# piotrkawa/audio-deepfake-adversarial-attacks

Hardware: AMD Instinct MI355X
Metric: adversarial utterances/sec, PGD-40 LCNN+LFCC 4s@16kHz (higher is better)
Workload: dtype f32

## Files before the change

### audio_deepfake_adversarial_attacks_amd/_lib.py

```python
from __future__ import annotations

import ctypes
from pathlib import Path

import os

_LIB_PATH = Path(os.environ.get("ADVSTEP_LIB") or Path(__file__).resolve().parent / "libadvstep.so")
_lib = None

OK, EINVAL, EWORKSPACE, ELAUNCH, ENODEVICE = 0, 1, 2, 3, 4
ABI_VERSION = 3

_p, _i64, _f32, _f64, _u64, _sz = (ctypes.c_void_p, ctypes.c_int64, ctypes.c_float, ctypes.c_double,
                                   ctypes.c_uint64, ctypes.c_size_t)

SIGNATURES = {
    "advstep_abi_version": (ctypes.c_int, []),
    "advstep_status_string": (ctypes.c_char_p, [ctypes.c_int]),
    "advstep_device_count": (ctypes.c_int, []),
    "advstep_row_workspace_bytes": (_sz, [_i64, _i64]),
    "advstep_minmax_normalize_f32": (ctypes.c_int, [_p, _p, _p, _p, _i64, _i64, _p, _sz, _p]),
    "advstep_minmax_revert_f32": (ctypes.c_int, [_p, _p, _p, _p, _i64, _i64, _p]),
    "advstep_fgsm_step_f32": (ctypes.c_int, [_p, _p, _p, _i64, _f32, _f32, _f32, _p]),
    "advstep_pgd_linf_init_noise_f32": (ctypes.c_int, [_p, _p, _p, _i64, _f32, _f32, _p]),
    "advstep_pgd_linf_init_philox_f32": (ctypes.c_int, [_p, _p, _i64, _f32, _f32, _f32, _u64, _u64, _p]),
# ... 24 lines not shown
    "advstep_lstm_backward_f32": (ctypes.c_int, [_p, _p, _p, _p, _p, _i64, _i64, _i64, _i64, _p]),
    "advstep_lstm_backward_bcast_f32": (ctypes.c_int, [_p, _p, _p, _p, _p, _i64, _i64, _i64, _i64, _p]),
    "advstep_lstm_backward_outer_f32": (ctypes.c_int, [_p, _p, _p, _p, _p, _p, _i64, _i64, _i64, _i64, _p]),
    "advstep_lcnn_tail_pack_f32": (ctypes.c_int, [_p, _p, _i64, _i64, _i64, _i64, _p]),
    "advstep_lcnn_tail_forward_f32": (ctypes.c_int, [_p, _p, _p, _p, _p, _i64, _i64, _i64, _p]),
    "advstep_lcnn_tail_unpack_add_f32": (ctypes.c_int, [_p, _p, _p, _i64, _i64, _i64, _i64, _p]),
    "advstep_lcnn_tail_unpack_add_outer_f32": (ctypes.c_int, [_p, _p, _p, _p, _i64, _i64, _i64, _i64, _p]),
    "advstep_gru_supported": (ctypes.c_int, [_i64]),
    "advstep_gru_forward_f32": (ctypes.c_int, [_p, _p, _p, _p, _p, _i64, _i64, _i64, _i64, _p]),
    "advstep_gru_backward_f32": (ctypes.c_int, [_p, _p, _p, _p, _p, _i64, _i64, _i64, _i64, _p]),
    "advstep_conv3x3_supported": (ctypes.c_int, [_i64, _i64]),
    "advstep_conv3x3_prepared_floats": (_sz, [_i64, _i64, ctypes.c_int]),
    "advstep_conv3x3_prepare_f32": (ctypes.c_int, [_p, _p, _p, _i64, _i64, ctypes.c_int, _p]),
    "advstep_conv3x3_mfm_pool2_forward_f32": (ctypes.c_int, [_p, _p, _p, _p, _p, _p, _p, _i64, _i64, _i64, _i64, _i64, _p]),
    "advstep_conv3x3_mfm_pool2_backward_f32": (ctypes.c_int, [_p, _p, _p, _p, _i64, _i64, _i64, _i64, _i64, _p]),
    "advstep_conv3x3_mfm_sel_bytes": (_sz, [_i64, _i64, _i64, _i64]),
    "advstep_conv3x3_mfm_forward_f32": (ctypes.c_int, [_p, _p, _p, _p, _p, _p, _p, _i64, _i64, _i64, _i64, _i64, _p]),
    "advstep_conv3x3_mfm_backward_f32": (ctypes.c_int, [_p, _p, _p, _p, _i64, _i64, _i64, _i64, _p]),
    "advstep_conv3x3_backward_data_f32": (ctypes.c_int, [_p, _p, _p, _i64, _i64, _i64, _i64, _i64, _p]),
    "advstep_afms_row_f32": (ctypes.c_int, [ctypes.c_int, _p, _p, _p, _p, _p, _p, _i64, _i64, _i64, _p]),
    "advstep_gate_maxpool2_backward_gate_f32": (ctypes.c_int, [_p, _p, _p, _p, _i64, _i64, _i64, _i64, _p]),
    "advstep_gate_maxpool2_backward_input_f32": (ctypes.c_int, [_p, _p, _p, _p, _p, _i64, _i64, _i64, _i64, _p]),
    "advstep_weighted_stats_forward_f32": (ctypes.c_int, [_p, _p, _p, _p, _i64, _i64, _p]),
    "advstep_weighted_stats_backward_f32": (ctypes.c_int, [_p, _p, _p, _p, _p, _p, _i64, _i64, _p]),
    "advstep_log_meannorm_max_length": (ctypes.c_int, []),
    "advstep_log_meannorm_forward_f32": (ctypes.c_int, [_p, ctypes.c_float, _p, _i64, _i64, _p]),
    "advstep_log_meannorm_backward_f32": (ctypes.c_int, [_p, _p, ctypes.c_float, _p, _i64, _i64, _p]),
    "advstep_tail_pool1d_forward_f32": (ctypes.c_int, [_p, _p, _p, _p, _p, _p, _p, _i64, _i64, _i64, _i64, _p]),
    "advstep_tail_pool1d_backward_f32": (ctypes.c_int, [_p, _p, _p, _p, _p, _p, _p, _i64, _i64, _i64, _i64, _p]),
    "advstep_res2net_link_forward_f32": (ctypes.c_int, [_p, _p, _p, _p, _p, _i64, _p, _i64, _p, _i64, _i64, _i64, _p]),
# ... 129 lines not shown
```

### audio_deepfake_adversarial_attacks_amd/csrc/advstep.hip

```cpp

#include <hip/hip_runtime.h>
#include <atomic>
#include <math.h>
#include <stdint.h>
#include <stdlib.h>

#include "advstep.h"
#include "advstep_common.h"
#include "row_tiles.h"

namespace {

constexpr int kMaxGrid = 256 * 16;

__device__ __forceinline__ float fgsm_elem(float x, float g, float eps, float lo, float hi) {
    return clampf(x + eps * sgn(g), lo, hi);
}

__device__ __forceinline__ float pgd_linf_elem(float a, float g, float x, float alpha, float eps, float lo,
                                               float hi) {
    a = a + alpha * sgn(g);
    float d = clampf(a - x, -eps, eps);
    return clampf(x + d, lo, hi);
}
// ... 790 lines not shown
                hipLaunchKernelGGL((KERNEL<false>), dim3(C_, (unsigned)nb_), dim3(kWgThreads), 0, st, __VA_ARGS__); \
        }                                                                                                  \
    } while (0)

extern "C" {

int advstep_abi_version(void) { return ADVSTEP_ABI_VERSION; }

const char *advstep_status_string(int status) {
    switch (status) {
        case ADVSTEP_OK: return "ok";
        case ADVSTEP_EINVAL: return "invalid argument";
        case ADVSTEP_EWORKSPACE: return "row workspace missing, misaligned or too small";
        case ADVSTEP_ELAUNCH: return "HIP kernel launch failed";
        case ADVSTEP_ENODEVICE: return "no HIP device";
        default: return "unknown status";
    }
}

int advstep_device_count(void) {
    int n = 0;
    if (hipGetDeviceCount(&n) != hipSuccess) {
        (void)hipGetLastError();
        return 0;
    }
    return n;
}

size_t advstep_row_workspace_bytes(int64_t B, int64_t T) {
    if (B <= 0 || T <= 0) return 0;
// ... 257 lines not shown
```

### audio_deepfake_adversarial_attacks_amd/csrc/lcnn_wino.hip

```cpp

#include <hip/hip_runtime.h>
#include <math.h>
#include <stdint.h>
#include <stdlib.h>

#include <type_traits>

#include "advstep_detector.h"
#include "advstep_lcnn.h"
#include "advstep_common.h"
#include "lcnn_wino_plan.h"

namespace {

extern __shared__ __attribute__((aligned(16))) float wino_u_s[];
__shared__ __attribute__((aligned(16))) float wino_cst[48];
__shared__ float wino_few_w[64];

__device__ __forceinline__ void weight_transform(const float (&g)[3][3], float (&u)[4][4]) {
    float t[4][3];
#pragma unroll
    for (int b = 0; b < 3; ++b) {
        t[0][b] = g[0][b];
        t[1][b] = 0.5f * (g[0][b] + g[1][b] + g[2][b]);
        t[2][b] = 0.5f * (g[0][b] - g[1][b] + g[2][b]);
        t[3][b] = g[2][b];
    }
#pragma unroll
    for (int a = 0; a < 4; ++a) {
        u[a][0] = t[a][0];
        u[a][1] = 0.5f * (t[a][0] + t[a][1] + t[a][2]);
        u[a][2] = 0.5f * (t[a][0] - t[a][1] + t[a][2]);
// ... 126 lines not shown
#pragma unroll
            for (int i = 0; i < kChunkFloats / 4 / kThreads; ++i) dst[threadIdx.x + i * kThreads] = src[threadIdx.x + i * kThreads];
        }
    }
    __device__ __forceinline__ void landed() const {
        if (DMA) __builtin_amdgcn_s_waitcnt(0x0F70);
    }
    __device__ __forceinline__ const float *a_ptr(int s, int buf, int g, int nl) const {
        return wino_u_s + buf * kChunkFloats + (((s & 3) * 4 + g) * 16 + nl) * 2;
    }
};

template <Epi EPI>
__device__ __forceinline__ void stage_constants(int slice, int Cout, const float *bias, const float *bn_mean,
                                                const float *bn_invstd, const GenArgs &ga) {
    if (adds_few(EPI) && threadIdx.x >= 64 && threadIdx.x < 128) {
        const float *w1x1 = bn_mean;
        const int i = threadIdx.x - 64, row = i >> 1, c = i & 1, ch = slice * 32 + row;
        wino_few_w[i] = (ch < Cout && c < ga.few) ? w1x1[ch * ga.few + c] : 0.0f;
    }
    if (has_constants(EPI) && threadIdx.x < 48) {
        const int q = threadIdx.x >> 4, j = threadIdx.x & 15;
        float v = q == 2 ? 1.0f : 0.0f;
        if (is_mfm(EPI)) {
            const int ch = slice * 16 + j;
            if (ch < Cout) {
                if (q == 2) v = bn_mean ? bn_invstd[ch] : 1.0f;
                else v = (bias ? bias[ch + q * Cout] : 0.0f) - (bn_mean ? bn_mean[ch] : 0.0f);
            }
        } else if (q < 2) {
// ... 20 lines not shown
        v[a4][2] = tr[a4][2] - tr[a4][1];
        v[a4][3] = tr[a4][1] - tr[a4][3];
    }
}

template <Epi EPI, bool STREAM, Src SRC, int NT = 2, bool GEN = false, bool WODD = false>
__global__ __launch_bounds__(kThreads) void wino3x3_kernel(const float *__restrict__ x, const uint8_t *__restrict__ xsel,
                                                           const float *__restrict__ U,
                                                           const float *__restrict__ bias,
                                                           const float *__restrict__ bn_mean,
                                                           const float *__restrict__ bn_invstd, float *__restrict__ y,
                                                           EpiBytes<EPI> *__restrict__ idx, int N, int K, int H, int W, int Cout,
                                                           int slices, int ranges, int slice0, GenArgs ga) {
    static_assert(NT == 2 || plain_store(EPI), "one accumulator tile only for the plain-store epilogues");
    static_assert(!GEN || SRC != Src::MfmPooled, "the general reduction reads dense tensors or a plain pooled gradient");
    const WgPlace wg = place_of_workgroup<NT>(slices, ranges, slice0, ga);
    const int half = wg.half, slice = wg.slice, range = wg.range;
    const int chunks = (K + kChunkCin - 1) / kChunkCin, steps = K / 4;
    const float *Usl = U + (int64_t)slice * chunks * kChunkFloats;
    const WeightChunks<STREAM && chunks_by_dma(SRC)> wc{Usl};
    constexpr bool kHasConst = has_constants(EPI);
    stage_constants<EPI>(slice, Cout, bias, bn_mean, bn_invstd, ga);
    if (!STREAM) {
        for (int c = 0; c < chunks; ++c) wc.copy(c, c);
    }
    if (!STREAM || kHasConst) __syncthreads();
    const int wave = threadIdx.x >> 6, lane = threadIdx.x & 63, g = lane >> 4, nl = lane & 15;
    const int TH = (H + 1) >> 1, TW = (W + 1) >> 1;
    const int tiles = N * TH * TW, groups = (tiles + 15) >> 4;
    const int iters = (groups + ranges * kWaves - 1) / (ranges * kWaves);
    const uint32_t plane = (uint32_t)(H * W);
    const int Hs = H >> 1, Ws = W >> 1, Cs = SRC == Src::MfmPooled ? K >> 1 : (GEN ? ga.Kreal : K);
    const uint32_t cplane = (uint32_t)(Hs * Ws);
    const int KA = GEN ? ga.K1 : K, KB = GEN ? ga.Kreal - ga.K1 : 0;
    const size_t src_elems = SRC == Src::Dense ? (size_t)N * KA * plane : (size_t)N * Cs * cplane;
    const __amdgpu_buffer_rsrc_t xr =
        __builtin_amdgcn_make_buffer_rsrc(const_cast<float *>(x), 0, (int)(src_elems * 4), 0x00020000);
    const __amdgpu_buffer_rsrc_t xr2 = __builtin_amdgcn_make_buffer_rsrc(
        const_cast<float *>(GEN && KB > 0 ? ga.x2 : x), 0, GEN && KB > 0 ? (int)((size_t)N * KB * plane * 4) : 0, 0x00020000);
    const __amdgpu_buffer_rsrc_t sr =
        __builtin_amdgcn_make_buffer_rsrc(const_cast<uint8_t *>(SRC != Src::Dense ? xsel : reinterpret_cast<const uint8_t *>(x)), 0,
// ... 238 lines not shown
                    }
                }
        }
        uint32_t hb[reads_sign_bytes(EPI) ? 4 : 1][reads_sign_bytes(EPI) ? NT : 1];
        if constexpr (reads_sign_bytes(EPI)) {
            const uint8_t *act = idx;
#pragma unroll
            for (int r = 0; r < 4; ++r)
#pragma unroll
                for (int m = 0; m < NT; ++m) {
                    const int ch = slice * 32 + (m + half) * 16 + 4 * g + r;
                    const bool live = valid && ch < Cout;
                    hb[r][m] = live ? act[(((size_t)n * Cout + ch) * TH + th) * TW + tw] : 0u;
                }
        }
        float xf[adds_few(EPI) ? 2 : 1][2][2];
        if constexpr (adds_few(EPI)) {
#pragma unroll
            for (int c = 0; c < 2; ++c) {
                xf[c][0][0] = xf[c][0][1] = xf[c][1][0] = xf[c][1][1] = 0.0f;
                if (valid && c < ga.few && th < (H >> 1) && tw < (W >> 1)) {
                    const float *xp = ga.x2 + (((size_t)n * ga.few + c) * H + 2 * th) * W + 2 * tw;
                    if ((W & 1) == 0) {
                        const f32x2 a = *reinterpret_cast<const f32x2 *>(xp), b2 = *reinterpret_cast<const f32x2 *>(xp + W);
                        xf[c][0][0] = a.x, xf[c][0][1] = a.y, xf[c][1][0] = b2.x, xf[c][1][1] = b2.y;
                    } else {
                        xf[c][0][0] = xp[0], xf[c][0][1] = xp[1], xf[c][1][0] = xp[W], xf[c][1][1] = xp[W + 1];
                    }
                }
            }
// ... 64 lines not shown
                            yy[m][e >> 1][e & 1] = fmaf(w1, xf[1][e >> 1][e & 1], fmaf(w0, xf[0][e >> 1][e & 1], yy[m][e >> 1][e & 1]));
                    }
                    float best = -INFINITY;
                    int code = 0;
#pragma unroll
                    for (int e = 0; e < 4; ++e) {
                        const float v = yy[m][e >> 1][e & 1];
                        if (v > best || v != v) { best = v; code = e; }
                    }
                    if (valid && live && th < Ho && tw < Wo) {
                        const size_t o = ((size_t)n * Cout + ch) * Ho * Wo + (size_t)th * Wo + tw;
                        y[o] = best;
                        idx[o] = (uint8_t)code;
                    }
                }
            } else {
#pragma unroll
                for (int m = 0; m < NT; ++m) {
                    const int ch = slice * 32 + (m + half) * 16 + 4 * g + r;
                    if (!(valid && ch < Cout)) continue;
                    if constexpr (EPI == Epi::ShiftLrelu) {
                        uint32_t bits = 0;
#pragma unroll
                        for (int e = 0; e < 4; ++e) {
                            const float v = yy[m][e >> 1][e & 1];
                            bits |= (uint32_t)(v > 0.0f) << e;
                            yy[m][e >> 1][e & 1] = v > 0.0f ? v : v * ga.slope;
                        }
                        if (idx) {
                            if (2 * tw + 1 >= W) bits &= 0x5u;
// ... 12 lines not shown
                        for (int e = 0; e < 4; ++e) yy[m][e >> 1][e & 1] *= (hb[r][m] >> e) & 1u ? 1.0f : ga.slope;
                    }
                    if ((W & 1) == 0) {
                        *reinterpret_cast<f32x2 *>(o) = (f32x2){yy[m][0][0], yy[m][0][1]};
                        if (h1) *reinterpret_cast<f32x2 *>(o + W) = (f32x2){yy[m][1][0], yy[m][1][1]};
                    } else {
                        const bool w1 = 2 * tw + 1 < W;
                        o[0] = yy[m][0][0];
                        if (w1) o[1] = yy[m][0][1];
                        if (h1) {
                            o[W] = yy[m][1][0];
                            if (w1) o[W + 1] = yy[m][1][1];
                        }
                    }
                }
            }
        }
    }
}

__global__ __launch_bounds__(256) void wino_mfm_backward_kernel(const float *__restrict__ gy, const uint8_t *__restrict__ sel,
                                                                const float *__restrict__ gscale, float *__restrict__ gout,
                                                                int C, int H, int W, int64_t total) {
    const int TH = (H + 1) >> 1, TW = (W + 1) >> 1;
    for (int64_t i = (int64_t)blockIdx.x * blockDim.x + threadIdx.x; i < total; i += (int64_t)gridDim.x * blockDim.x) {
        const int w = (int)(i % W), h = (int)((i / W) % H);
        const int64_t nc = i / ((int64_t)W * H);
        const int c = (int)(nc % C);
        const int64_t n = nc / C;
        const uint32_t bits = sel[(nc * TH + (h >> 1)) * TW + (w >> 1)];
// ... 111 lines not shown
                                               (int)ceil_div(Cin, 32), as_stream(stream));
}

int advstep_conv3x3_mfm_pool2_backward_f32(const float *gy, const uint8_t *idx, const float *U, float *gx, int64_t N,
                                           int64_t Cin, int64_t C, int64_t H, int64_t W, advstep_stream_t stream) {
    ADVSTEP_REQUIRE(N >= 0 && H >= 0 && W >= 0 && advstep_conv3x3_supported(Cin, 2 * C));
    if (N == 0 || H == 0 || W == 0) return ADVSTEP_OK;
    ADVSTEP_REQUIRE(gx);
    if (H / 2 == 0 || W / 2 == 0)
        return hipMemsetAsync(gx, 0, (size_t)N * Cin * H * W * sizeof(float), as_stream(stream)) == hipSuccess ? ADVSTEP_OK
                                                                                                               : ADVSTEP_ELAUNCH;
    ADVSTEP_REQUIRE(gy && idx && U);
    ADVSTEP_REQUIRE(wino_sizes_ok(N, H, W, 0, C, 0));
    return launch_wino<Epi::Store, Src::MfmPooled>(gy, idx, U, nullptr, nullptr, nullptr, gx, nullptr, N, 2 * C, H, W, Cin,
                                                   (int)ceil_div(Cin, 32), as_stream(stream));
}


int advstep_resconv_supported(int64_t K1, int64_t K2, int64_t rows) {
    return K1 >= 1 && K2 >= 0 && (K2 == 0 || K1 % 4 == 0) && K1 + K2 <= 256 && rows >= 1 && rows <= 256;
}

size_t advstep_resconv_prepared_floats(int64_t K1, int64_t K2, int64_t rows) {
    if (!advstep_resconv_supported(K1, K2, rows)) return 0;
    return (size_t)(ceil_div(rows, 32) * ceil_div(K1 + K2, kChunkCin) * kChunkFloats);
}

int advstep_resconv_prepare_f32(const float *w3, const float *w1, const float *rscale, const float *kscale, float *U,
                                int64_t rows, int64_t K1, int64_t K2, int transpose, advstep_stream_t stream) {
    ADVSTEP_REQUIRE(w3 && U && advstep_resconv_supported(K1, K2, rows) && (K2 == 0 || w1) && (transpose == 0 || transpose == 1));
// ... 92 lines not shown
```

### audio_deepfake_adversarial_attacks_amd/csrc/lcnn_wino_plan.h

```cpp
#pragma once

#include <stdint.h>
#include <stdlib.h>

#include <type_traits>

#include "advstep_common.h"

namespace {

constexpr int kWaves = 8, kThreads = kWaves * 64;
constexpr int kChunkCin = 16;
constexpr int kChunkFloats = 16 * kChunkCin * 32;
constexpr int kMaxResident = 4;
constexpr int kComputeUnits = 256;

enum class Src : int {
    Dense = 0,
    MfmPooled = 1,
    Pooled = 2,
};

enum class Epi : int {
    Store = 0,
    MfmPoolBn = 1,
    MfmBn = 2,
    ShiftLrelu = 3,
    BiasPool = 4,
    LreluGradH = 5,
    LreluGradBytes = 6,
    BiasPoolFew = 7,
};

constexpr bool is_mfm(Epi e) { return e == Epi::MfmPoolBn || e == Epi::MfmBn; }
constexpr bool adds_few(Epi e) { return e == Epi::BiasPoolFew; }
constexpr bool pools(Epi e) { return e == Epi::MfmPoolBn || e == Epi::BiasPool || adds_few(e); }
constexpr bool reads_sign_bytes(Epi e) { return e == Epi::LreluGradBytes; }
constexpr bool has_constants(Epi e) { return is_mfm(e) || e == Epi::ShiftLrelu || e == Epi::BiasPool || adds_few(e); }
constexpr bool plain_store(Epi e) { return !is_mfm(e) && !pools(e); }

constexpr bool chunks_by_dma(Src s) {
#ifdef WINO_GLDS
    return WINO_GLDS;
#else
    return s == Src::MfmPooled;
#endif
}

template <Epi EPI>
using EpiBytes = std::conditional_t<reads_sign_bytes(EPI), const uint8_t, uint8_t>;

struct WinoKnobs {
    bool half_slice;
    bool halves;
    bool xcd;
    int range_mult;
};

inline WinoKnobs read_wino_knobs() {
    auto not_off = [](const char *name) {
        const char *e = getenv(name);
        return !(e && e[0] == '0');
    };
    const char *em = getenv("ADVSTEP_WINO_RANGE_MULT");
    return {not_off("ADVSTEP_WINO_HALF_SLICE"), not_off("ADVSTEP_WINO_HALVES"), not_off("ADVSTEP_WINO_XCD"),
            em && em[0] >= '1' && em[0] <= '8' ? em[0] - '0' : 1};
}

struct WinoLaunch {
    int NT;
    bool stream, wodd;
    int halves, n_slices, slice0, ranges, xcd;
    size_t lds;
};
struct WinoPlan {
    int count = 0;
    WinoLaunch launch[2];
};

inline WinoPlan plan_wino(Epi epi, Src src, bool gen, int64_t N, int64_t K, int64_t H, int64_t W, int64_t Cout, int slices,
                          const WinoKnobs &knobs) {
// ... 42 lines not shown
```

### audio_deepfake_adversarial_attacks_amd/lcnn_ops.py

```python
from __future__ import annotations

from typing import Optional

import torch

from . import _lib
from .hip_ops import _Launch, _require, _stream


def _gemm(fn, a2d: torch.Tensor, b2d: torch.Tensor, *lead):
    with _Launch("rnn_projection_gemm", a2d.device, work=2.0 * a2d.shape[0] * a2d.shape[1] * b2d.shape[1]):
        return fn(*lead, a2d, b2d)


def _check_input(x: torch.Tensor, bias: Optional[torch.Tensor]):
    _require(x, "x")
    if x.dim() != 4 or x.shape[1] % 2 != 0:
        raise ValueError(f"expected a contiguous (N, 2C, H, W) tensor, got {tuple(x.shape)}")
    if bias is not None:
        _require(bias, "bias")
        if bias.numel() != x.shape[1]:
            raise ValueError(f"bias must have {x.shape[1]} entries, got {bias.numel()}")


# ... 110 lines not shown
        with _Launch("conv5_mfm_pool2_backward", gy.device, work=12.5 * N * C * H * W, tensors=(gy, idx, gx)):
            st = _lib.load().advstep_conv5_mfm_pool2_backward_f32(gy.data_ptr(), idx.data_ptr(), weight.data_ptr(),
                                                                  gx.data_ptr(), N, C, H, W, _stream(gy.device))
        _lib.check(st, "advstep_conv5_mfm_pool2_backward_f32")
        return gx, None, None


def conv5_mfm_pool2(x: torch.Tensor, weight: torch.Tensor, bias: Optional[torch.Tensor] = None) -> torch.Tensor:
    return _Conv5MfmPool2.apply(x.contiguous(), weight.contiguous(), bias)


class _Conv1x1Mfm(torch.autograd.Function):

    @staticmethod
    def forward(ctx, x, weight, bias, bn):
        _require(x, "x"), _require(weight, "weight")
        if bias is not None:
            _require(bias, "bias")
        bn_mean, bn_invstd = _bn_ptrs(bn)
        if x.dim() != 4 or weight.dim() != 4 or tuple(weight.shape[2:]) != (1, 1) or weight.shape[1] != x.shape[1] \
                or weight.shape[0] % 2 != 0 or (bias is not None and bias.numel() != weight.shape[0]):
            raise ValueError(f"expected x (N, Cin, H, W), weight (2C, Cin, 1, 1), bias (2C); got {tuple(x.shape)}, "
                             f"{tuple(weight.shape)}")
        N, Cin, H, W = x.shape
        C, P = weight.shape[0] // 2, H * W
        lib = _lib.load()
        if not lib.advstep_conv1x1_mfm_supported(Cin):
            raise ValueError(f"conv1x1_mfm supports Cin in (32, 48, 64), got {Cin}")
        y = torch.empty((N, C, H, W), dtype=x.dtype, device=x.device)
        sel = torch.empty(max(lib.advstep_conv1x1_mfm_sel_bytes(N, C, P), 4), dtype=torch.uint8, device=x.device)
        with _Launch("conv1x1_mfm_forward", x.device, work=4.0 * N * Cin * C * P, tensors=(x, y, sel)):
            st = lib.advstep_conv1x1_mfm_forward_f32(x.data_ptr(), weight.data_ptr(),
                                                     bias.data_ptr() if bias is not None else None, bn_mean, bn_invstd,
                                                     y.data_ptr(), sel.data_ptr(), N, Cin, C, P, _stream(x.device))
        _lib.check(st, "advstep_conv1x1_mfm_forward_f32")
        ctx.save_for_backward(sel, weight, *([bn[1]] if bn is not None else []))
        ctx.shape = (N, Cin, C, H, W)
        return y

    @staticmethod
    def backward(ctx, gy):
        if ctx.needs_input_grad[1] or (len(ctx.needs_input_grad) > 2 and ctx.needs_input_grad[2]):
            raise RuntimeError("conv1x1_mfm provides the input gradient only; call it with frozen weights "
                               "(the model falls back to Conv2d + mfm otherwise)")
        sel, weight, *scale = ctx.saved_tensors
        N, Cin, C, H, W = ctx.shape
        gy = gy.contiguous()
        gx = torch.empty((N, Cin, H, W), dtype=gy.dtype, device=gy.device)
        with _Launch("conv1x1_mfm_backward", gy.device, work=4.0 * N * Cin * C * H * W, tensors=(gy, sel, gx)):
            st = _lib.load().advstep_conv1x1_mfm_backward_f32(gy.data_ptr(), sel.data_ptr(), weight.data_ptr(),
                                                              scale[0].data_ptr() if scale else None, gx.data_ptr(), N, Cin,
                                                              C, H * W, _stream(gy.device))
        _lib.check(st, "advstep_conv1x1_mfm_backward_f32")
        return gx, None, None, None


def conv1x1_mfm_supported(in_channels: int) -> bool:
    return bool(_lib.load().advstep_conv1x1_mfm_supported(in_channels))


def conv1x1_mfm(x: torch.Tensor, weight: torch.Tensor, bias: Optional[torch.Tensor] = None, bn=None) -> torch.Tensor:
    return _Conv1x1Mfm.apply(x.contiguous(), weight.contiguous(), bias, bn)



def _prepared_weights(weight: torch.Tensor, mode: int, gscale: Optional[torch.Tensor] = None) -> torch.Tensor:
    cache = getattr(weight, "_advstep_wino", None)
    if cache is None or cache[0] != (weight._version, weight.data_ptr()):
        cache = ((weight._version, weight.data_ptr()), {})
        try:
            weight._advstep_wino = cache
        except AttributeError:
            pass
    slot = (mode, None if gscale is None else (gscale.data_ptr(), gscale._version))
    U = cache[1].get(slot)
    if U is None:
        Cout, Cin = weight.shape[0], weight.shape[1]
# ... 7 lines not shown
            cache[1].clear()
        cache[1][slot] = (U, gscale)
        return U
    return U[0]


def _batch_chunks(N: int, per_sample_floats: int):
    step = max(1, ((1 << 31) - 1) // (4 * per_sample_floats))
    return [(lo, min(N, lo + step)) for lo in range(0, N, step)]


class _Conv3x3MfmPool2(torch.autograd.Function):

    @staticmethod
    def forward(ctx, x, weight, bias, bn, U, U_grad):
        _require(x, "x"), _require(weight, "weight")
        if bias is not None:
            _require(bias, "bias")
        N, Cin, H, W = x.shape
        C = weight.shape[0] // 2
        bn_mean, bn_invstd = _bn_ptrs(bn)
        y = torch.empty((N, C, H // 2, W // 2), dtype=x.dtype, device=x.device)
        idx = torch.empty(max(y.numel(), 2), dtype=torch.uint8, device=x.device)
        lib = _lib.load()
        per_out = C * (H // 2) * (W // 2)
        for lo, hi in _batch_chunks(N, max(Cin * H * W, 1)):
            with _Launch("conv3x3_mfm_pool2_forward", x.device, work=16.0 * (hi - lo) * C * Cin * H * W):
                st = lib.advstep_conv3x3_mfm_pool2_forward_f32(
                    x[lo:hi].data_ptr(), U.data_ptr(), bias.data_ptr() if bias is not None else None, bn_mean, bn_invstd,
                    y[lo:hi].data_ptr() if hi > lo else None, idx.data_ptr() + lo * per_out, hi - lo, Cin, C, H, W,
                    _stream(x.device))
            _lib.check(st, "advstep_conv3x3_mfm_pool2_forward_f32")
        ctx.save_for_backward(idx, U_grad)
        ctx.shape = (N, Cin, C, H, W)
        return y

    @staticmethod
    def backward(ctx, gy):
        idx, U = ctx.saved_tensors
        N, Cin, C, H, W = ctx.shape
        gy = gy.contiguous()
        lib = _lib.load()
        gx = torch.empty((N, Cin, H, W), dtype=gy.dtype, device=gy.device)
        per_cell = C * (H // 2) * (W // 2)
        for lo, hi in _batch_chunks(N, max(4 * per_cell, Cin * H * W, 1)):
            with _Launch("conv3x3_mfm_pool2_backward", gy.device, work=16.0 * (hi - lo) * C * Cin * H * W):
                st = lib.advstep_conv3x3_mfm_pool2_backward_f32(gy[lo:hi].data_ptr(), idx.data_ptr() + lo * per_cell,
                                                                U.data_ptr(), gx[lo:hi].data_ptr(), hi - lo, Cin, C, H, W,
                                                                _stream(gy.device))
            _lib.check(st, "advstep_conv3x3_mfm_pool2_backward_f32")
        return gx, None, None, None, None, None


class _Conv3x3Mfm(torch.autograd.Function):

    @staticmethod
    def forward(ctx, x, weight, bias, bn, U, U_grad):
        _require(x, "x"), _require(weight, "weight")
        if bias is not None:
            _require(bias, "bias")
        N, Cin, H, W = x.shape
        C = weight.shape[0] // 2
        bn_mean, bn_invstd = _bn_ptrs(bn)
        lib = _lib.load()
        y = torch.empty((N, C, H, W), dtype=x.dtype, device=x.device)
        per_sel = C * ((H + 1) // 2) * ((W + 1) // 2)
# ... 27 lines not shown
            _lib.check(st, "advstep_conv3x3_backward_data_f32")
        return gx, None, None, None, None, None


def conv3x3_mfm(x: torch.Tensor, weight: torch.Tensor, bias: Optional[torch.Tensor] = None, bn=None) -> torch.Tensor:
    weight = weight if weight.is_contiguous() else weight.contiguous()
    return _Conv3x3Mfm.apply(x.contiguous(), weight, bias, bn, _prepared_weights(weight, 0), _prepared_weights(weight, 1))


def conv3x3_supported(in_channels: int, out_channels: int) -> bool:
    return bool(_lib.load().advstep_conv3x3_supported(in_channels, out_channels))


def conv3x3_mfm_pool2(x: torch.Tensor, weight: torch.Tensor, bias: Optional[torch.Tensor] = None, bn=None) -> torch.Tensor:
    weight = weight if weight.is_contiguous() else weight.contiguous()
    return _Conv3x3MfmPool2.apply(x.contiguous(), weight, bias, bn, _prepared_weights(weight, 0),
                                  _prepared_weights(weight, 2, None if bn is None else bn[1]))



class _LstmLayer(torch.autograd.Function):

    @staticmethod
    def forward(ctx, x, w_ih, w_hh, bias):
        _require(x, "x"), _require(w_ih, "w_ih"), _require(w_hh, "w_hh"), _require(bias, "bias")
        T, B, I = x.shape
        D, H4, H = w_hh.shape
        if H4 != 4 * H or tuple(w_ih.shape) != (D * H4, I) or bias.numel() != D * H4:
            raise ValueError("inconsistent LSTM parameter shapes")
        gx = _gemm(torch.addmm, x.reshape(T * B, I), w_ih.t(), bias)
        out = torch.empty((T, B, D * H), dtype=x.dtype, device=x.device)
        gates = torch.empty((T, B, D, H4), dtype=x.dtype, device=x.device)
# ... 194 lines not shown
```

### include/advstep.h

```cpp
#ifndef ADVSTEP_H_
#define ADVSTEP_H_

#include <stddef.h>
#include <stdint.h>

#ifdef __cplusplus
extern "C" {
#endif

#define ADVSTEP_ABI_VERSION 3

enum {
    ADVSTEP_OK = 0,
    ADVSTEP_EINVAL = 1,
    ADVSTEP_EWORKSPACE = 2,
    ADVSTEP_ELAUNCH = 3,
    ADVSTEP_ENODEVICE = 4
};

typedef void *advstep_stream_t;


int advstep_abi_version(void);
const char *advstep_status_string(int status);
int advstep_device_count(void);
size_t advstep_row_workspace_bytes(int64_t B, int64_t T);


int advstep_minmax_normalize_f32(const float *x, float *x01, float *mn, float *mx, int64_t B, int64_t T,
                                 void *ws, size_t ws_bytes, advstep_stream_t stream);

int advstep_minmax_revert_f32(const float *x01, const float *mn, const float *mx, float *out, int64_t B,
// ... 54 lines not shown
```

### include/advstep_lcnn.h

```cpp
#ifndef ADVSTEP_LCNN_H_
#define ADVSTEP_LCNN_H_

#include <stddef.h>
#include <stdint.h>

#include "advstep.h"

#ifdef __cplusplus
extern "C" {
#endif

size_t advstep_mfm_sel_bytes(int64_t N, int64_t C, int64_t HW);

int advstep_mfm_forward_f32(const float *x, const float *bias, const float *bn_mean, const float *bn_invstd, float *y,
                            uint8_t *sel, int64_t N, int64_t C, int64_t HW, advstep_stream_t stream);

int advstep_mfm_backward_f32(const float *gy, const uint8_t *sel, const float *gscale, float *gx, int64_t N, int64_t C,
                             int64_t HW, advstep_stream_t stream);

int advstep_mfm_pool2_forward_f32(const float *x, const float *bias, const float *bn_mean, const float *bn_invstd,
                                  float *y, uint8_t *idx, int64_t N, int64_t C, int64_t H, int64_t W,
                                  advstep_stream_t stream);

int advstep_mfm_pool2_backward_f32(const float *gy, const uint8_t *idx, const float *gscale, float *gx, int64_t N,
// ... 24 lines not shown
                                          int64_t C, int64_t H, int64_t W, advstep_stream_t stream);

size_t advstep_conv3x3_mfm_sel_bytes(int64_t N, int64_t C, int64_t H, int64_t W);
int advstep_conv3x3_mfm_forward_f32(const float *x, const float *U, const float *bias, const float *bn_mean,
                                    const float *bn_invstd, float *y, uint8_t *sel, int64_t N, int64_t Cin, int64_t C,
                                    int64_t H, int64_t W, advstep_stream_t stream);
int advstep_conv3x3_mfm_backward_f32(const float *gy, const uint8_t *sel, const float *gscale, float *gout, int64_t N,
                                     int64_t C, int64_t H, int64_t W, advstep_stream_t stream);

int advstep_conv3x3_backward_data_f32(const float *gout, const float *U, float *gx, int64_t N, int64_t Cin, int64_t Cout,
                                      int64_t H, int64_t W, advstep_stream_t stream);

int advstep_conv3x3_mfm_pool2_backward_f32(const float *gy, const uint8_t *idx, const float *U, float *gx, int64_t N,
                                           int64_t Cin, int64_t C, int64_t H, int64_t W, advstep_stream_t stream);

int advstep_lstm_supported(int64_t H);
int advstep_lstm_forward_f32(const float *gx, const float *w_hh, float *out, float *gates, float *cell, int64_t T,
                             int64_t B, int64_t D, int64_t H, advstep_stream_t stream);

int advstep_lstm_backward_f32(const float *dout, const float *w_hh, const float *gates, const float *cell, float *dgx,
                              int64_t T, int64_t B, int64_t D, int64_t H, advstep_stream_t stream);
int advstep_lstm_backward_bcast_f32(const float *dout_row, const float *w_hh, const float *gates, const float *cell,
                                    float *dgx, int64_t T, int64_t B, int64_t D, int64_t H, advstep_stream_t stream);
int advstep_lstm_backward_outer_f32(const float *dz, const float *row, const float *w_hh, const float *gates, const float *cell,
                                    float *dgx, int64_t T, int64_t B, int64_t D, int64_t H, advstep_stream_t stream);

int advstep_lcnn_tail_pack_f32(const float *x4, float *xt, int64_t B, int64_t C, int64_t T, int64_t W, advstep_stream_t stream);
int advstep_lcnn_tail_forward_f32(const float *a, const float *xt, const float *w, const float *bias, float *z, int64_t T,
                                  int64_t B, int64_t F, advstep_stream_t stream);
int advstep_lcnn_tail_unpack_add_f32(const float *dxt, const float *g0, float *dx4, int64_t B, int64_t C, int64_t T, int64_t W,
// ... 15 lines not shown
```

Before: 2050.

## Fold conv1x1-MFM input gradient into Winograd conv3x3-MFM-pool2 backward epilogue

Adds a Conv1x1MfmGrad epilogue to the Winograd conv3x3 backward kernel. After producing the 32-channel gradient tile, the kernel applies the preceding 64x32 1x1 conv's MFM selection mask and BN scale and runs the 1x1 transpose matmul with MFMA in registers, writing the final input gradient directly. The Python side detects a conv1x1_mfm output feeding conv3x3_mfm_pool2 and routes both layers through a combined autograd function. This removes the intermediate gradient write and read plus one launch per pair. In exchange it adds register and LDS pressure, and it falls back to the two separate kernels when the shape is unsupported.

```diff
diff --git a/audio_deepfake_adversarial_attacks_amd/_lib.py b/audio_deepfake_adversarial_attacks_amd/_lib.py
--- a/audio_deepfake_adversarial_attacks_amd/_lib.py
+++ b/audio_deepfake_adversarial_attacks_amd/_lib.py
@@ -8,7 +8,7 @@
 _LIB_PATH = Path(os.environ.get("ADVSTEP_LIB") or Path(__file__).resolve().parent / "libadvstep.so")
 _lib = None
 
-OK, EINVAL, EWORKSPACE, ELAUNCH, ENODEVICE = 0, 1, 2, 3, 4
+OK, EINVAL, EWORKSPACE, ELAUNCH, ENODEVICE, EUNSUPPORTED = 0, 1, 2, 3, 4, 5
 ABI_VERSION = 3
 
 _p, _i64, _f32, _f64, _u64, _sz = (ctypes.c_void_p, ctypes.c_int64, ctypes.c_float, ctypes.c_double,
@@ -63,6 +63,7 @@
     "advstep_conv3x3_prepare_f32": (ctypes.c_int, [_p, _p, _p, _i64, _i64, ctypes.c_int, _p]),
     "advstep_conv3x3_mfm_pool2_forward_f32": (ctypes.c_int, [_p, _p, _p, _p, _p, _p, _p, _i64, _i64, _i64, _i64, _i64, _p]),
     "advstep_conv3x3_mfm_pool2_backward_f32": (ctypes.c_int, [_p, _p, _p, _p, _i64, _i64, _i64, _i64, _i64, _p]),
+    "advstep_conv3x3_mfm_pool2_backward_conv1x1_f32": (ctypes.c_int, [_p, _p, _p, _p, _p, _p, _p, _i64, _i64, _i64, _i64, _i64, _p]),
     "advstep_conv3x3_mfm_sel_bytes": (_sz, [_i64, _i64, _i64, _i64]),
     "advstep_conv3x3_mfm_forward_f32": (ctypes.c_int, [_p, _p, _p, _p, _p, _p, _p, _i64, _i64, _i64, _i64, _i64, _p]),
     "advstep_conv3x3_mfm_backward_f32": (ctypes.c_int, [_p, _p, _p, _p, _i64, _i64, _i64, _i64, _p]),
diff --git a/audio_deepfake_adversarial_attacks_amd/csrc/advstep.hip b/audio_deepfake_adversarial_attacks_amd/csrc/advstep.hip
--- a/audio_deepfake_adversarial_attacks_amd/csrc/advstep.hip
+++ b/audio_deepfake_adversarial_attacks_amd/csrc/advstep.hip
@@ -828,6 +828,7 @@
         case ADVSTEP_EWORKSPACE: return "row workspace missing, misaligned or too small";
         case ADVSTEP_ELAUNCH: return "HIP kernel launch failed";
         case ADVSTEP_ENODEVICE: return "no HIP device";
+        case ADVSTEP_EUNSUPPORTED: return "shape not supported by this entry point";
         default: return "unknown status";
     }
 }
diff --git a/audio_deepfake_adversarial_attacks_amd/csrc/lcnn_wino.hip b/audio_deepfake_adversarial_attacks_amd/csrc/lcnn_wino.hip
--- a/audio_deepfake_adversarial_attacks_amd/csrc/lcnn_wino.hip
+++ b/audio_deepfake_adversarial_attacks_amd/csrc/lcnn_wino.hip
@@ -16,6 +16,7 @@
 extern __shared__ __attribute__((aligned(16))) float wino_u_s[];
 __shared__ __attribute__((aligned(16))) float wino_cst[48];
 __shared__ float wino_few_w[64];
+__shared__ float wino_w1x1[64 * 32];
 
 __device__ __forceinline__ void weight_transform(const float (&g)[3][3], float (&u)[4][4]) {
     float t[4][3];
@@ -172,6 +173,16 @@
 template <Epi EPI>
 __device__ __forceinline__ void stage_constants(int slice, int Cout, const float *bias, const float *bn_mean,
                                                 const float *bn_invstd, const GenArgs &ga) {
+    if constexpr (folds_conv1x1(EPI)) {
+        const float *w1x1 = bias, *gscale = bn_mean;
+#pragma unroll
+        for (int j = 0; j < 64 * 32 / kThreads; ++j) {
+            const int i = threadIdx.x + j * kThreads;
+            const int nl = i & 15, g = (i >> 4) & 3, rt = (i >> 6) & 1, r = (i >> 7) & 3, m = (i >> 9) & 1, h = i >> 10;
+            wino_w1x1[i] = w1x1[(h * 32 + m * 16 + 4 * g + r) * 32 + rt * 16 + nl];
+        }
+        if (threadIdx.x < 32) wino_cst[threadIdx.x] = gscale ? gscale[threadIdx.x] : 1.0f;
+    }
     if (adds_few(EPI) && threadIdx.x >= 64 && threadIdx.x < 128) {
         const float *w1x1 = bn_mean;
         const int i = threadIdx.x - 64, row = i >> 1, c = i & 1, ch = slice * 32 + row;
@@ -222,6 +233,7 @@
                                                            int slices, int ranges, int slice0, GenArgs ga) {
     static_assert(NT == 2 || plain_store(EPI), "one accumulator tile only for the plain-store epilogues");
     static_assert(!GEN || SRC != Src::MfmPooled, "the general reduction reads dense tensors or a plain pooled gradient");
+    static_assert(!folds_conv1x1(EPI) || (NT == 2 && SRC == Src::MfmPooled), "the folded 1x1 gradient: one full slice of a pooled block");
     const WgPlace wg = place_of_workgroup<NT>(slices, ranges, slice0, ga);
     const int half = wg.half, slice = wg.slice, range = wg.range;
     const int chunks = (K + kChunkCin - 1) / kChunkCin, steps = K / 4;
@@ -232,7 +244,7 @@
     if (!STREAM) {
         for (int c = 0; c < chunks; ++c) wc.copy(c, c);
     }
-    if (!STREAM || kHasConst) __syncthreads();
+    if (!STREAM || kHasConst || folds_conv1x1(EPI)) __syncthreads();
     const int wave = threadIdx.x >> 6, lane = threadIdx.x & 63, g = lane >> 4, nl = lane & 15;
     const int TH = (H + 1) >> 1, TW = (W + 1) >> 1;
     const int tiles = N * TH * TW, groups = (tiles + 15) >> 4;
@@ -501,6 +513,20 @@
                     hb[r][m] = live ? act[(((size_t)n * Cout + ch) * TH + th) * TW + tw] : 0u;
                 }
         }
+        uint32_t selw[folds_conv1x1(EPI) ? 4 : 1];
+        float bv[folds_conv1x1(EPI) ? 2 : 1][folds_conv1x1(EPI) ? 4 : 1][4];
+        float a1x1[folds_conv1x1(EPI) ? 16 : 1][2];
+        if constexpr (folds_conv1x1(EPI)) {
+            const uint32_t words = ((plane + 31u) >> 5) << 5;
+            const __amdgpu_buffer_rsrc_t mr =
+                __builtin_amdgcn_make_buffer_rsrc(const_cast<uint8_t *>(idx), 0, (int)((uint32_t)N * words * 4u), 0x00020000);
+            const uint32_t m_off = ((uint32_t)n * words + (uint32_t)(2 * th * W + 2 * tw)) * 4u;
+            const uint32_t dr = 2 * th + 1 < H ? (uint32_t)W * 4u : 0u, dc = 2 * tw + 1 < W ? 4u : 0u;
+            const int sh = 16 * (g & 1) + 4 * (g >> 1);
+#pragma unroll
+            for (int e = 0; e < 4; ++e)
+                selw[e] = __builtin_amdgcn_raw_buffer_load_b32(mr, m_off + (e >> 1 ? dr : 0u) + (e & 1 ? dc : 0u), 0, 0) >> sh;
+        }
         float xf[adds_few(EPI) ? 2 : 1][2][2];
         if constexpr (adds_few(EPI)) {
 #pragma unroll
@@ -595,6 +621,19 @@
                         idx[o] = (uint8_t)code;
                     }
                 }
+            } else if constexpr (folds_conv1x1(EPI)) {
+#pragma unroll
+                for (int m = 0; m < 2; ++m)
+#pragma unroll
+                    for (int e = 0; e < 4; ++e) bv[m][r][e] = yy[m][e >> 1][e & 1] * wino_cst[m * 16 + 4 * g + r];
+                if (r == 1) {
+#pragma unroll
+                    for (int ks = 0; ks < 16; ++ks) {
+                        a1x1[ks][0] = wino_w1x1[lane + (2 * ks) * 64];
+                        a1x1[ks][1] = wino_w1x1[lane + (2 * ks + 1) * 64];
+                    }
+                    __builtin_amdgcn_sched_barrier(0);
+                }
             } else {
 #pragma unroll
                 for (int m = 0; m < NT; ++m) {
@@ -637,6 +676,46 @@
                         }
                     }
                 }
+            }
+        }
+        if constexpr (folds_conv1x1(EPI)) {
+            const f32x4 zero = {0.0f, 0.0f, 0.0f, 0.0f};
+            f32x4 out[4][2] = {{zero, zero}, {zero, zero}, {zero, zero}, {zero, zero}};
+            __builtin_amdgcn_s_setprio(1);
+#pragma unroll
+            for (int hm = 0; hm < 4; ++hm)
+#pragma unroll
+                for (int r = 0; r < 4; ++r) {
+                    const int h = hm >> 1, m = hm & 1;
+                    const float a0 = a1x1[hm * 4 + r][0], a1 = a1x1[hm * 4 + r][1];
+#pragma unroll
+                    for (int e = 0; e < 4; ++e) {
+                        const float b = ((selw[e] >> (r + 8 * m)) & 1u) == (uint32_t)h ? bv[m][r][e] : 0.0f;
+                        out[e][0] = __builtin_amdgcn_mfma_f32_16x16x4f32(a0, b, out[e][0], 0, 0, 0);
+                        out[e][1] = __builtin_amdgcn_mfma_f32_16x16x4f32(a1, b, out[e][1], 0, 0, 0);
+                    }
+                }
+            __builtin_amdgcn_s_setprio(0);
+            if (valid) {
+                const bool h1 = 2 * th + 1 < H, w1 = 2 * tw + 1 < W;
+#pragma unroll
+                for (int rt = 0; rt < 2; ++rt)
+#pragma unroll
+                    for (int r = 0; r < 4; ++r) {
+                        const int ch = rt * 16 + 4 * g + r;
+                        float *o = y + (((size_t)n * Cout + ch) * H + 2 * th) * W + 2 * tw;
+                        if ((W & 1) == 0) {
+                            *reinterpret_cast<f32x2 *>(o) = (f32x2){out[0][rt][r], out[1][rt][r]};
+                            if (h1) *reinterpret_cast<f32x2 *>(o + W) = (f32x2){out[2][rt][r], out[3][rt][r]};
+                        } else {
+                            o[0] = out[0][rt][r];
+                            if (w1) o[1] = out[1][rt][r];
+                            if (h1) {
+                                o[W] = out[2][rt][r];
+                                if (w1) o[W + 1] = out[3][rt][r];
+                            }
+                        }
+                    }
             }
         }
     }
@@ -778,6 +857,31 @@
     ADVSTEP_REQUIRE(wino_sizes_ok(N, H, W, 0, C, 0));
     return launch_wino<Epi::Store, Src::MfmPooled>(gy, idx, U, nullptr, nullptr, nullptr, gx, nullptr, N, 2 * C, H, W, Cin,
                                                    (int)ceil_div(Cin, 32), as_stream(stream));
+}
+
+int advstep_conv3x3_mfm_pool2_backward_conv1x1_f32(const float *gy, const uint8_t *idx, const float *U, const float *w1x1,
+                                                   const void *sel1x1, const float *gscale1x1, float *gx, int64_t N, int64_t Cin,
+                                                   int64_t C, int64_t H, int64_t W, advstep_stream_t stream) {
+    ADVSTEP_REQUIRE(N >= 0 && H >= 0 && W >= 0 && advstep_conv3x3_supported(Cin, 2 * C));
+    const WinoKnobs knobs = read_wino_knobs();
+    if (Cin != 32 || !knobs.fuse_1x1) return ADVSTEP_EUNSUPPORTED;
+    if (N == 0 || H == 0 || W == 0) return ADVSTEP_OK;
+    ADVSTEP_REQUIRE(gx);
+    if (H / 2 == 0 || W / 2 == 0)
+        return hipMemsetAsync(gx, 0, (size_t)N * Cin * H * W * sizeof(float), as_stream(stream)) == hipSuccess ? ADVSTEP_OK
+                                                                                                               : ADVSTEP_ELAUNCH;
+    ADVSTEP_REQUIRE(gy && idx && U && w1x1 && sel1x1 && (reinterpret_cast<uintptr_t>(sel1x1) & 3u) == 0);
+    ADVSTEP_REQUIRE(wino_sizes_ok(N, H, W, 0, C, 0) && (uint64_t)N * (uint64_t)(ceil_div(H * W, 32) * 32) * 4 < (1ull << 31));
+    const WinoPlan plan = plan_wino(Epi::Store, Src::MfmPooled, false, N, 2 * C, H, W, Cin, 1, knobs);
+    if (plan.count != 1 || plan.launch[0].NT != 2 || plan.launch[0].halves || plan.launch[0].n_slices != 1) return ADVSTEP_EUNSUPPORTED;
+    const WinoLaunch &l = plan.launch[0];
+    const auto kernel = l.stream ? wino3x3_kernel<Epi::Conv1x1MfmGrad, true, Src::MfmPooled, 2, false, false>
+                                 : wino3x3_kernel<Epi::Conv1x1MfmGrad, false, Src::MfmPooled, 2, false, false>;
+    (void)hipFuncSetAttribute(reinterpret_cast<const void *>(kernel), hipFuncAttributeMaxDynamicSharedMemorySize, (int)l.lds);
+    hipLaunchKernelGGL(kernel, dim3((unsigned)l.ranges), dim3(kThreads), l.lds, as_stream(stream), gy, idx, U, w1x1, gscale1x1,
+                       (const float *)nullptr, gx, const_cast<uint8_t *>(static_cast<const uint8_t *>(sel1x1)), (int)N, (int)(2 * C), (int)H, (int)W, (int)Cin,
+                       1, l.ranges, 0, GenArgs{nullptr, 0, 0, 1.0f, l.xcd, 0, 0});
+    return status_after_launch();
 }
 
 
diff --git a/audio_deepfake_adversarial_attacks_amd/csrc/lcnn_wino_plan.h b/audio_deepfake_adversarial_attacks_amd/csrc/lcnn_wino_plan.h
--- a/audio_deepfake_adversarial_attacks_amd/csrc/lcnn_wino_plan.h
+++ b/audio_deepfake_adversarial_attacks_amd/csrc/lcnn_wino_plan.h
@@ -30,12 +30,14 @@
     LreluGradH = 5,
     LreluGradBytes = 6,
     BiasPoolFew = 7,
+    Conv1x1MfmGrad = 8,
 };
 
 constexpr bool is_mfm(Epi e) { return e == Epi::MfmPoolBn || e == Epi::MfmBn; }
 constexpr bool adds_few(Epi e) { return e == Epi::BiasPoolFew; }
 constexpr bool pools(Epi e) { return e == Epi::MfmPoolBn || e == Epi::BiasPool || adds_few(e); }
 constexpr bool reads_sign_bytes(Epi e) { return e == Epi::LreluGradBytes; }
+constexpr bool folds_conv1x1(Epi e) { return e == Epi::Conv1x1MfmGrad; }
 constexpr bool has_constants(Epi e) { return is_mfm(e) || e == Epi::ShiftLrelu || e == Epi::BiasPool || adds_few(e); }
 constexpr bool plain_store(Epi e) { return !is_mfm(e) && !pools(e); }
 
@@ -55,6 +57,7 @@
     bool halves;
     bool xcd;
     int range_mult;
+    bool fuse_1x1;
 };
 
 inline WinoKnobs read_wino_knobs() {
@@ -64,7 +67,7 @@
     };
     const char *em = getenv("ADVSTEP_WINO_RANGE_MULT");
     return {not_off("ADVSTEP_WINO_HALF_SLICE"), not_off("ADVSTEP_WINO_HALVES"), not_off("ADVSTEP_WINO_XCD"),
-            em && em[0] >= '1' && em[0] <= '8' ? em[0] - '0' : 1};
+            em && em[0] >= '1' && em[0] <= '8' ? em[0] - '0' : 1, not_off("ADVSTEP_WINO_FUSE_1X1_GRAD")};
 }
 
 struct WinoLaunch {
diff --git a/audio_deepfake_adversarial_attacks_amd/lcnn_ops.py b/audio_deepfake_adversarial_attacks_amd/lcnn_ops.py
--- a/audio_deepfake_adversarial_attacks_amd/lcnn_ops.py
+++ b/audio_deepfake_adversarial_attacks_amd/lcnn_ops.py
@@ -148,28 +148,8 @@
 
     @staticmethod
     def forward(ctx, x, weight, bias, bn):
-        _require(x, "x"), _require(weight, "weight")
-        if bias is not None:
-            _require(bias, "bias")
-        bn_mean, bn_invstd = _bn_ptrs(bn)
-        if x.dim() != 4 or weight.dim() != 4 or tuple(weight.shape[2:]) != (1, 1) or weight.shape[1] != x.shape[1] \
-                or weight.shape[0] % 2 != 0 or (bias is not None and bias.numel() != weight.shape[0]):
-            raise ValueError(f"expected x (N, Cin, H, W), weight (2C, Cin, 1, 1), bias (2C); got {tuple(x.shape)}, "
-                             f"{tuple(weight.shape)}")
-        N, Cin, H, W = x.shape
-        C, P = weight.shape[0] // 2, H * W
-        lib = _lib.load()
-        if not lib.advstep_conv1x1_mfm_supported(Cin):
-            raise ValueError(f"conv1x1_mfm supports Cin in (32, 48, 64), got {Cin}")
-        y = torch.empty((N, C, H, W), dtype=x.dtype, device=x.device)
-        sel = torch.empty(max(lib.advstep_conv1x1_mfm_sel_bytes(N, C, P), 4), dtype=torch.uint8, device=x.device)
-        with _Launch("conv1x1_mfm_forward", x.device, work=4.0 * N * Cin * C * P, tensors=(x, y, sel)):
-            st = lib.advstep_conv1x1_mfm_forward_f32(x.data_ptr(), weight.data_ptr(),
-                                                     bias.data_ptr() if bias is not None else None, bn_mean, bn_invstd,
-                                                     y.data_ptr(), sel.data_ptr(), N, Cin, C, P, _stream(x.device))
-        _lib.check(st, "advstep_conv1x1_mfm_forward_f32")
+        y, sel, ctx.shape = _conv1x1_mfm_forward(x, weight, bias, bn)
         ctx.save_for_backward(sel, weight, *([bn[1]] if bn is not None else []))
-        ctx.shape = (N, Cin, C, H, W)
         return y
 
     @staticmethod
@@ -178,15 +158,40 @@
             raise RuntimeError("conv1x1_mfm provides the input gradient only; call it with frozen weights "
                                "(the model falls back to Conv2d + mfm otherwise)")
         sel, weight, *scale = ctx.saved_tensors
-        N, Cin, C, H, W = ctx.shape
-        gy = gy.contiguous()
-        gx = torch.empty((N, Cin, H, W), dtype=gy.dtype, device=gy.device)
-        with _Launch("conv1x1_mfm_backward", gy.device, work=4.0 * N * Cin * C * H * W, tensors=(gy, sel, gx)):
-            st = _lib.load().advstep_conv1x1_mfm_backward_f32(gy.data_ptr(), sel.data_ptr(), weight.data_ptr(),
-                                                              scale[0].data_ptr() if scale else None, gx.data_ptr(), N, Cin,
-                                                              C, H * W, _stream(gy.device))
-        _lib.check(st, "advstep_conv1x1_mfm_backward_f32")
-        return gx, None, None, None
+        return _conv1x1_mfm_backward(gy.contiguous(), sel, weight, scale[0].data_ptr() if scale else None, ctx.shape), None, None, None
+
+
+def _conv1x1_mfm_forward(x, weight, bias, bn):
+    _require(x, "x"), _require(weight, "weight")
+    if bias is not None:
+        _require(bias, "bias")
+    bn_mean, bn_invstd = _bn_ptrs(bn)
+    if x.dim() != 4 or weight.dim() != 4 or tuple(weight.shape[2:]) != (1, 1) or weight.shape[1] != x.shape[1] \
+            or weight.shape[0] % 2 != 0 or (bias is not None and bias.numel() != weight.shape[0]):
+        raise ValueError(f"expected x (N, Cin, H, W), weight (2C, Cin, 1, 1), bias (2C); got {tuple(x.shape)}, "
+                         f"{tuple(weight.shape)}")
+    N, Cin, H, W = x.shape
+    C, P = weight.shape[0] // 2, H * W
+    lib = _lib.load()
+    if not lib.advstep_conv1x1_mfm_supported(Cin):
+        raise ValueError(f"conv1x1_mfm supports Cin in (32, 48, 64), got {Cin}")
+    y = torch.empty((N, C, H, W), dtype=x.dtype, device=x.device)
+    sel = torch.empty(max(lib.advstep_conv1x1_mfm_sel_bytes(N, C, P), 4), dtype=torch.uint8, device=x.device)
+    with _Launch("conv1x1_mfm_forward", x.device, work=4.0 * N * Cin * C * P, tensors=(x, y, sel)):
+        st = lib.advstep_conv1x1_mfm_forward_f32(x.data_ptr(), weight.data_ptr(), bias.data_ptr() if bias is not None else None,
+                                                 bn_mean, bn_invstd, y.data_ptr(), sel.data_ptr(), N, Cin, C, P, _stream(x.device))
+    _lib.check(st, "advstep_conv1x1_mfm_forward_f32")
+    return y, sel, (N, Cin, C, H, W)
+
+
+def _conv1x1_mfm_backward(gy, sel, weight, gscale_ptr, shape):
+    N, Cin, C, H, W = shape
+    gx = torch.empty((N, Cin, H, W), dtype=gy.dtype, device=gy.device)
+    with _Launch("conv1x1_mfm_backward", gy.device, work=4.0 * N * Cin * C * H * W, tensors=(gy, sel, gx)):
+        st = _lib.load().advstep_conv1x1_mfm_backward_f32(gy.data_ptr(), sel.data_ptr(), weight.data_ptr(), gscale_ptr, gx.data_ptr(),
+                                                          N, Cin, C, H * W, _stream(gy.device))
+    _lib.check(st, "advstep_conv1x1_mfm_backward_f32")
+    return gx
 
 
 def conv1x1_mfm_supported(in_channels: int) -> bool:
@@ -194,7 +199,12 @@
 
 
 def conv1x1_mfm(x: torch.Tensor, weight: torch.Tensor, bias: Optional[torch.Tensor] = None, bn=None) -> torch.Tensor:
-    return _Conv1x1Mfm.apply(x.contiguous(), weight.contiguous(), bias, bn)
+    x, weight = x.contiguous(), weight.contiguous()
+    y = _Conv1x1Mfm.apply(x, weight, bias, bn)
+    if y.requires_grad and x.requires_grad and tuple(weight.shape[:2]) == (64, 32):
+        sel, _, *scale = y.grad_fn.saved_tensors
+        y._advstep_conv1x1 = (x, sel, weight, scale[0] if scale else None)
+    return y
 
 
 
@@ -232,42 +242,80 @@
 
     @staticmethod
     def forward(ctx, x, weight, bias, bn, U, U_grad):
-        _require(x, "x"), _require(weight, "weight")
-        if bias is not None:
-            _require(bias, "bias")
-        N, Cin, H, W = x.shape
-        C = weight.shape[0] // 2
-        bn_mean, bn_invstd = _bn_ptrs(bn)
-        y = torch.empty((N, C, H // 2, W // 2), dtype=x.dtype, device=x.device)
-        idx = torch.empty(max(y.numel(), 2), dtype=torch.uint8, device=x.device)
-        lib = _lib.load()
-        per_out = C * (H // 2) * (W // 2)
-        for lo, hi in _batch_chunks(N, max(Cin * H * W, 1)):
-            with _Launch("conv3x3_mfm_pool2_forward", x.device, work=16.0 * (hi - lo) * C * Cin * H * W):
-                st = lib.advstep_conv3x3_mfm_pool2_forward_f32(
-                    x[lo:hi].data_ptr(), U.data_ptr(), bias.data_ptr() if bias is not None else None, bn_mean, bn_invstd,
-                    y[lo:hi].data_ptr() if hi > lo else None, idx.data_ptr() + lo * per_out, hi - lo, Cin, C, H, W,
-                    _stream(x.device))
-            _lib.check(st, "advstep_conv3x3_mfm_pool2_forward_f32")
+        y, idx, ctx.shape = _conv3x3_mfm_pool2_forward(x, weight, bias, bn, U)
         ctx.save_for_backward(idx, U_grad)
-        ctx.shape = (N, Cin, C, H, W)
         return y
 
     @staticmethod
     def backward(ctx, gy):
         idx, U = ctx.saved_tensors
-        N, Cin, C, H, W = ctx.shape
+        return _conv3x3_mfm_pool2_backward(gy.contiguous(), idx, U, ctx.shape), None, None, None, None, None
+
+
+def _conv3x3_mfm_pool2_forward(x, weight, bias, bn, U):
+    _require(x, "x"), _require(weight, "weight")
+    if bias is not None:
+        _require(bias, "bias")
+    N, Cin, H, W = x.shape
+    C = weight.shape[0] // 2
+    bn_mean, bn_invstd = _bn_ptrs(bn)
+    y = torch.empty((N, C, H // 2, W // 2), dtype=x.dtype, device=x.device)
+    idx = torch.empty(max(y.numel(), 2), dtype=torch.uint8, device=x.device)
+    lib = _lib.load()
+    per_out = C * (H // 2) * (W // 2)
+    for lo, hi in _batch_chunks(N, max(Cin * H * W, 1)):
+        with _Launch("conv3x3_mfm_pool2_forward", x.device, work=16.0 * (hi - lo) * C * Cin * H * W):
+            st = lib.advstep_conv3x3_mfm_pool2_forward_f32(
+                x[lo:hi].data_ptr(), U.data_ptr(), bias.data_ptr() if bias is not None else None, bn_mean, bn_invstd,
+                y[lo:hi].data_ptr() if hi > lo else None, idx.data_ptr() + lo * per_out, hi - lo, Cin, C, H, W, _stream(x.device))
+        _lib.check(st, "advstep_conv3x3_mfm_pool2_forward_f32")
+    return y, idx, (N, Cin, C, H, W)
+
+
+def _conv3x3_mfm_pool2_backward(gy, idx, U, shape):
+    N, Cin, C, H, W = shape
+    lib = _lib.load()
+    gx = torch.empty((N, Cin, H, W), dtype=gy.dtype, device=gy.device)
+    per_cell = C * (H // 2) * (W // 2)
+    for lo, hi in _batch_chunks(N, max(4 * per_cell, Cin * H * W, 1)):
+        with _Launch("conv3x3_mfm_pool2_backward", gy.device, work=16.0 * (hi - lo) * C * Cin * H * W):
+            st = lib.advstep_conv3x3_mfm_pool2_backward_f32(gy[lo:hi].data_ptr(), idx.data_ptr() + lo * per_cell, U.data_ptr(),
+                                                            gx[lo:hi].data_ptr(), hi - lo, Cin, C, H, W, _stream(gy.device))
+        _lib.check(st, "advstep_conv3x3_mfm_pool2_backward_f32")
+    return gx
+
+
+class _Conv1x1MfmConv3x3MfmPool2(torch.autograd.Function):
+
+    @staticmethod
+    def forward(ctx, x0, h, sel1, w1, scale1, weight, bias, bn, U, U_grad):
+        y, idx, shape3 = _conv3x3_mfm_pool2_forward(h, weight, bias, bn, U)
+        ctx.save_for_backward(idx, U_grad, sel1, w1, *([scale1] if scale1 is not None else []))
+        ctx.shape = ((x0.shape[0], w1.shape[1], w1.shape[0] // 2, x0.shape[2], x0.shape[3]), shape3)
+        return y
+
+    @staticmethod
+    def backward(ctx, gy):
+        if any(ctx.needs_input_grad[1:]):
+            raise RuntimeError("conv3x3_mfm_pool2 behind conv1x1_mfm provides the input gradient only; call it with frozen weights")
+        idx3, U, sel1, w1, *scale1 = ctx.saved_tensors
+        (N, Cin1, C1, H, W), (_, Cin3, C3, _, _) = ctx.shape
         gy = gy.contiguous()
         lib = _lib.load()
-        gx = torch.empty((N, Cin, H, W), dtype=gy.dtype, device=gy.device)
-        per_cell = C * (H // 2) * (W // 2)
-        for lo, hi in _batch_chunks(N, max(4 * per_cell, Cin * H * W, 1)):
-            with _Launch("conv3x3_mfm_pool2_backward", gy.device, work=16.0 * (hi - lo) * C * Cin * H * W):
-                st = lib.advstep_conv3x3_mfm_pool2_backward_f32(gy[lo:hi].data_ptr(), idx.data_ptr() + lo * per_cell,
-                                                                U.data_ptr(), gx[lo:hi].data_ptr(), hi - lo, Cin, C, H, W,
-                                                                _stream(gy.device))
-            _lib.check(st, "advstep_conv3x3_mfm_pool2_backward_f32")
-        return gx, None, None, None, None, None
+        gscale1 = scale1[0].data_ptr() if scale1 else None
+        st = _lib.EUNSUPPORTED
+        if len(_batch_chunks(N, max(4 * C3 * (H // 2) * (W // 2), Cin3 * H * W, 1))) == 1:
+            gx = torch.empty((N, Cin1, H, W), dtype=gy.dtype, device=gy.device)
+            with _Launch("conv3x3_mfm_pool2_backward", gy.device, work=16.0 * N * C3 * Cin3 * H * W + 4.0 * N * Cin1 * C1 * H * W):
+                st = lib.advstep_conv3x3_mfm_pool2_backward_conv1x1_f32(gy.data_ptr(), idx3.data_ptr(), U.data_ptr(), w1.data_ptr(),
+                                                                        sel1.data_ptr(), gscale1, gx.data_ptr(), N, Cin3, C3, H, W,
+                                                                        _stream(gy.device))
+        if st == _lib.EUNSUPPORTED:
+            gh = _conv3x3_mfm_pool2_backward(gy, idx3, U, (N, Cin3, C3, H, W))
+            gx = _conv1x1_mfm_backward(gh, sel1, w1, gscale1, (N, Cin1, C1, H, W))
+        else:
+            _lib.check(st, "advstep_conv3x3_mfm_pool2_backward_conv1x1_f32")
+        return (gx,) + (None,) * 9
 
 
 class _Conv3x3Mfm(torch.autograd.Function):
@@ -325,8 +373,12 @@
 
 def conv3x3_mfm_pool2(x: torch.Tensor, weight: torch.Tensor, bias: Optional[torch.Tensor] = None, bn=None) -> torch.Tensor:
     weight = weight if weight.is_contiguous() else weight.contiguous()
-    return _Conv3x3MfmPool2.apply(x.contiguous(), weight, bias, bn, _prepared_weights(weight, 0),
-                                  _prepared_weights(weight, 2, None if bn is None else bn[1]))
+    U, U_grad = _prepared_weights(weight, 0), _prepared_weights(weight, 2, None if bn is None else bn[1])
+    pair = getattr(x, "_advstep_conv1x1", None)
+    if pair is not None and weight.shape[1] == 32 and torch.is_grad_enabled() and pair[0].requires_grad:
+        x0, sel1, w1, scale1 = pair
+        return _Conv1x1MfmConv3x3MfmPool2.apply(x0, x.detach(), sel1, w1, scale1, weight, bias, bn, U, U_grad)
+    return _Conv3x3MfmPool2.apply(x.contiguous(), weight, bias, bn, U, U_grad)
 
 
 
diff --git a/include/advstep.h b/include/advstep.h
--- a/include/advstep.h
+++ b/include/advstep.h
@@ -15,7 +15,8 @@
     ADVSTEP_EINVAL = 1,
     ADVSTEP_EWORKSPACE = 2,
     ADVSTEP_ELAUNCH = 3,
-    ADVSTEP_ENODEVICE = 4
+    ADVSTEP_ENODEVICE = 4,
+    ADVSTEP_EUNSUPPORTED = 5
 };
 
 typedef void *advstep_stream_t;
diff --git a/include/advstep_lcnn.h b/include/advstep_lcnn.h
--- a/include/advstep_lcnn.h
+++ b/include/advstep_lcnn.h
@@ -62,6 +62,10 @@
 int advstep_conv3x3_mfm_pool2_backward_f32(const float *gy, const uint8_t *idx, const float *U, float *gx, int64_t N,
                                            int64_t Cin, int64_t C, int64_t H, int64_t W, advstep_stream_t stream);
 
+int advstep_conv3x3_mfm_pool2_backward_conv1x1_f32(const float *gy, const uint8_t *idx, const float *U, const float *w1x1,
+                                                   const void *sel1x1, const float *gscale1x1, float *gx, int64_t N,
+                                                   int64_t Cin, int64_t C, int64_t H, int64_t W, advstep_stream_t stream);
+
 int advstep_lstm_supported(int64_t H);
 int advstep_lstm_forward_f32(const float *gx, const float *w_hh, float *out, float *gates, float *cell, int64_t T,
                              int64_t B, int64_t D, int64_t H, advstep_stream_t stream);
```

Result: no change. 2069, median of 6 (+0.9%).
